# USCCACS/RXMD

Hardware: AMD Instinct MI355X
Metric: MD steps/sec (RDX, 979,776 atoms/GPU; one step advances every GPU's domain: weak scaling, wall-clock steps/s of the whole job) (higher is better)
Workload: dtype f64

## Files before the change

rxmd_amd/csrc/bonded.hip:

```cpp
#include "engine.h"

#include <hipcub/hipcub.hpp>

#include <algorithm>
#include <cstdlib>
#include <type_traits>

namespace rxmd {

static inline int nblk(long long n, int b) { return n > 0 ? static_cast<int>((n + b - 1) / b) : 1; }

static constexpr double MINBO0 = 1e-4, cutof2_esub = 1e-4;
static constexpr double MAXANGLE = 0.999999999999, MINANGLE = -0.999999999999, NSMALL = 1e-10;
static constexpr double PI_ = 3.14159265358979;

__device__ inline double wave_sum_b(double v) { return wave_sum64(v); }
__device__ inline void block_energy_add(double v, double *dst) {
  __shared__ double sm[8];
  v = wave_sum_b(v);
  const int w = threadIdx.x >> 6;
  __syncthreads();
  if ((threadIdx.x & 63) == 0) sm[w] = v;
  __syncthreads();
  if (threadIdx.x == 0) {
// ... 213 lines not shown
        const double BOjk_p4 = pow(BOjk, ap.pval4), exp3jk = exp(-aj.pval3 * BOjk_p4), fn7jk = 1.0 - exp3jk;
        const double exp7 = exp(-ap.pval7 * delta_ang), trm8 = 1.0 + exp6 + exp7;
        const double fn8j = aj.pval5 - (aj.pval5 - 1.0) * (2.0 + exp6) / trm8;
        const double theta0 = PI_ - ap.theta00 * (1.0 - ex10);
        const double theta_diff = theta0 - theta_ijk;
        const double exp2 = exp(-ap.pval2 * theta_diff * theta_diff);
        e5 += fn7ij * fn7jk * fn8j * (ap.pval1 - ap.pval1 * exp2);
        const double Cf7ij = aj.pval3 * ap.pval4 * (BOij_p4 / BOij) * exp3ij;
        const double Cf7jk = aj.pval3 * ap.pval4 * (BOjk_p4 / BOjk) * exp3jk;
        const double Cf8j = (1.0 - aj.pval5) / (trm8 * trm8) * (ff.pval6 * exp6 * trm8 - (2.0 + exp6) * (ff.pval6 * exp6 - ap.pval7 * exp7));
        const double Ctheta0 = ff.pval10 * ap.theta00 * ex10;
        const double CEval1 = Cf7ij * fn7jk * fn8j * ap.pval1 * (1.0 - exp2);
        const double CEval2 = fn7ij * Cf7jk * fn8j * ap.pval1 * (1.0 - exp2);
        const double CEval3 = fn7ij * fn7jk * Cf8j * ap.pval1 * (1.0 - exp2);
        const double CEval4 = 2.0 * ap.pval1 * ap.pval2 * fn7ij * fn7jk * fn8j * exp2 * theta_diff;
        const double CEval5 = CEval4 * Ctheta0 * CSBO2;
        const double CEval6 = CEval5 * dSBO1, CEval7 = CEval5 * dSBO2, CEval8 = CEval4 / sin_ijk;
        const double PEpen = ap.ppen1 * fn9 * epen[oi] * epen[ok];
        e6 += PEpen;
        const double CEpen1 = Cf9j / fn9 * PEpen, CEpen2 = -2.0 * ff.ppen2 * (BOij - 2.0) * PEpen, CEpen3 = -2.0 * ff.ppen2 * (BOjk - 2.0) * PEpen;
        const double sum_BOi = delta[i] + ff.atom[ti].Val, sum_BOk = delta[k] + ff.atom[tk].Val;
        const double ui = -BOij + sum_BOi, uk = -BOjk + sum_BOk;
        const double PEcoa = ap.pcoa1 / (1.0 + exp_coa2) * ecoa[oi] * ecoa[ok];
        e7 += PEcoa;
        const double CEcoa1 = -2.0 * ff.pcoa4 * (BOij - 1.5) * PEcoa, CEcoa2 = -2.0 * ff.pcoa4 * (BOjk - 1.5) * PEcoa;
        const double CEcoa3 = -ff.pcoa2 * exp_coa2 / (1.0 + exp_coa2) * PEcoa;
        const double CEcoa4 = -2.0 * ff.pcoa3 * ui * PEcoa, CEcoa5 = -2.0 * ff.pcoa3 * uk * PEcoa;
        ai_cf += CEpen2 + CEcoa1 - CEcoa4 + CEval1;
        acc1(cf1, l_cf, ok, CEpen3 + CEcoa2 - CEcoa5 + CEval2);
        S_d1 += CEpen1 + CEcoa3 + CEval3 + CEval7; S_v6 += CEval6; S_v5 += CEval5;
        ai_cd += CEcoa4; acc1(cdn, l_cd, ok, CEcoa5);
        V3 fi, fk;
        angle_forces(CEval8, rij, nij, rjk, njk, fi, fk);
        ai_fx += fi.x; ai_fy += fi.y; ai_fz += fi.z;
        acc1(fnx, l_fx, ok, fk.x); acc1(fny, l_fy, ok, fk.y); acc1(fnz, l_fz, ok, fk.z);
        fself.x -= fi.x + fk.x; fself.y -= fi.y + fk.y; fself.z -= fi.z + fk.z;
      }
      if (ai_cf != 0.0) acc1(cf1, l_cf, oi, ai_cf);
      if (ai_cd != 0.0) acc1(cdn, l_cd, oi, ai_cd);
      if (ai_fx != 0.0 || ai_fy != 0.0 || ai_fz != 0.0) { acc1(fnx, l_fx, oi, ai_fx); acc1(fny, l_fy, oi, ai_fy); acc1(fnz, l_fz, oi, ai_fz); }
    }
    if (S_d1 != 0.0 || S_v6 != 0.0 || S_v5 != 0.0)
      for (int n1 = 0; n1 < nj; ++n1) {
        const int o = ob + n1;
        acc1(cf1, l_cf, o, S_d1 + S_v6 * ipow7(bo0[o])); cf2[o] += S_v5; cf3[o] += S_v5;
      }
    fx[j] += fself.x; fy[j] += fself.y; fz[j] += fself.z;
  }
  wave_lds_sync();
  for (int t = lane_; t < nst; t += 64) { cf1[ob_w + t] = l_cf[t]; cdn[ob_w + t] = l_cd[t]; fnx[ob_w + t] = l_fx[t]; fny[ob_w + t] = l_fy[t]; fnz[ob_w + t] = l_fz[t]; }
  block_energy_add(e5, pe + 5); block_energy_add(e6, pe + 6); block_energy_add(e7, pe + 7);
}

constexpr int E3Q_BC = 192;
template <int MINW, int NA>
__global__ void __launch_bounds__(256, MINW) k_e3q(int N, int NG, DevFF ff, const int *__restrict__ boff, const int *__restrict__ nbr, const unsigned char *__restrict__ btype, const int *__restrict__ type,
                                              const double *__restrict__ x, const double *__restrict__ y, const double *__restrict__ z,
                                              const double *__restrict__ bo0, const double *__restrict__ bo2, const double *__restrict__ bo3,
                                              const double *__restrict__ delta, const double *__restrict__ nlp, const double *__restrict__ dDlp,
                                              const double *__restrict__ epen, const double *__restrict__ ecoa,
                                              double *__restrict__ cf1, double *__restrict__ cf2, double *__restrict__ cf3, double *__restrict__ cdn,
                                              double *__restrict__ fnx, double *__restrict__ fny, double *__restrict__ fnz,
                                              double *__restrict__ cds, double *__restrict__ fx, double *__restrict__ fy, double *__restrict__ fz, double *__restrict__ pe, int probe) {
  constexpr int E3Q_NA = NA, E3Q_MAXL = (E3Q_BC / NA < 32) ? E3Q_BC / NA : 32, LPA = 64 / NA;
  __shared__ unsigned char s_ix3[512];
  __shared__ double s_ang[64][7];
  __shared__ double s_c[4][16][12];
  __shared__ int s_ci[4][16][4];
  __shared__ double s_acc[4][5][E3Q_BC];
  __shared__ double s_at[4][16][3];
  __shared__ unsigned char s_cap[4][256], s_own[4][E3Q_BC];
  __shared__ float s_cbo[4][E3Q_BC];
  __shared__ unsigned short s_q[4][128];
  constexpr int CAPW = (256 / NA < 32) ? 256 / NA : 32;
  const int lane = threadIdx.x & 63, w = __builtin_amdgcn_readfirstlane(static_cast<int>(threadIdx.x >> 6));
  for (int t = threadIdx.x; t < ff.n1 * ff.n1 * ff.n1; t += 256) s_ix3[t] = static_cast<unsigned char>(ff.inxn3[t]);
  const bool ang_lds = ff.nvaty <= 63;
  if (ang_lds) for (int t = threadIdx.x; t < 7 * (ff.nvaty + 1); t += 256) s_ang[t / 7][t % 7] = reinterpret_cast<const double *>(ff.angle)[t];
  __syncthreads();
  double e5 = 0.0, e6 = 0.0, e7 = 0.0;
  for (int vb = blockIdx.x; vb < NG; vb += gridDim.x) {
  const int jbase = (xcd_swizzle(vb, NG) * 4 + w) * E3Q_NA;
  if (jbase >= N) continue;
  const int na = min(E3Q_NA, N - jbase);
  const int ob_w = boff[jbase], nb_w = boff[jbase + na] - ob_w;
  for (int r = lane; r < nb_w; r += 64) { s_acc[w][0][r] = bo0[ob_w + r]; s_acc[w][1][r] = bo2[ob_w + r] + bo3[ob_w + r]; }
  for (int t = lane; t < 3 * E3Q_BC; t += 64) (&s_acc[w][2][0])[t] = 0.0;
  if (lane < E3Q_NA) { s_at[w][lane][0] = 0.0; s_at[w][lane][1] = 0.0; s_at[w][lane][2] = 0.0; s_ci[w][lane][2] = 0; s_ci[w][lane][3] = 0; }
  wave_lds_sync();
  if (lane < na) {
    const int j = jbase + lane;
    const int tj = type[j], ob = boff[j], nj = min(boff[j + 1] - ob, E3Q_MAXL);
    const DevAtomP aj = ff.atom[tj];
    double sum_BO8 = 0.0, sum_SBO1 = 0.0;
    int nc = 0;
    for (int n1 = 0; n1 < nj; ++n1) {
      const int r = ob + n1 - ob_w;
      const double b = s_acc[w][0][r], b2 = b * b, b4 = b2 * b2;
      sum_BO8 -= b4 * b4;
      sum_SBO1 += s_acc[w][1][r];
      if (b - cutof2_esub > 0.0) { s_cbo[w][lane * E3Q_MAXL + nc] = static_cast<float>(b); s_cap[w][lane * CAPW + nc++] = static_cast<unsigned char>(n1); }
      s_own[w][r] = static_cast<unsigned char>(lane);
    }
    const double prod_SBO = exp(sum_BO8);
    const double dlj = delta[j];
    const double delta_ang = dlj + aj.Val - aj.Valangle;
    const double nlpj = nlp[j], dDj = dDlp[j];
    const double exp_pen3 = exp(-ff.ppen3 * dlj), exp_pen4 = exp(ff.ppen4 * dlj);
    const double trm34 = 1.0 + exp_pen3 + exp_pen4;
    const double fn9 = (2.0 + exp_pen3) / trm34;
    const double Cf9j = (-ff.ppen3 * exp_pen3 * trm34 - (2.0 + exp_pen3) * (-ff.ppen3 * exp_pen3 + ff.ppen4 * exp_pen4)) / (trm34 * trm34);
    const double delta_val = dlj + aj.Val - aj.Valval;
    const double SBO = sum_SBO1 + (1.0 - prod_SBO) * (-delta_ang - ff.pval8 * nlpj);
    double SBO2 = 0.0, CSBO2 = 0.0;
    if (SBO > 0.0 && SBO <= 1.0) { const double pw = exp(ff.pval9 * log(SBO)); SBO2 = pw; CSBO2 = ff.pval9 * (pw / SBO); }
    else if (SBO > 1.0 && SBO < 2.0) { const double b_ = 2.0 - SBO, pw = exp(ff.pval9 * log(b_)); SBO2 = 2.0 - pw; CSBO2 = ff.pval9 * (pw / b_); }
    else if (SBO >= 2.0) SBO2 = 2.0;
    double *c = s_c[w][lane];
    c[0] = x[j]; c[1] = y[j]; c[2] = z[j]; c[3] = delta_ang; c[4] = exp(ff.pval6 * delta_ang); c[5] = exp(-ff.pval10 * (2.0 - SBO2)); c[6] = CSBO2;
    c[7] = -8.0 * prod_SBO * (delta_ang + ff.pval8 * nlpj); c[8] = (prod_SBO - 1.0) * (1.0 - ff.pval8 * dDj); c[9] = fn9; c[10] = Cf9j / fn9; c[11] = exp(ff.pcoa2 * delta_val);
    s_ci[w][lane][0] = tj; s_ci[w][lane][1] = ob; s_ci[w][lane][2] = nj; s_ci[w][lane][3] = nc;
  }
  wave_lds_sync();
  for (int t = lane; t < 2 * E3Q_BC; t += 64) (&s_acc[w][0][0])[t] = 0.0;
  wave_lds_sync();
  int qn = 0, qh = 0;
  auto evaluate = [&](int cnt) {
#ifdef RXMD_EXPERIMENTS
    if (probe == 2) return;
    if (probe == 5) { if (lane == 0) { atomicAdd(pe + 5, 1.0); atomicAdd(pe + 6, static_cast<double>(cnt)); } return; }
#endif
    if (lane < cnt) {
      const int key = s_q[w][(qh + lane) & 127];
      const int a = key >> 10, i1 = (key >> 5) & 31, k1 = key & 31;
      const double *c = s_c[w][a];
      const int tj = s_ci[w][a][0], ob = s_ci[w][a][1];
      const int oi = ob + i1, ok = ob + k1;
      const double xj = c[0], yj = c[1], zj = c[2], delta_ang = c[3], exp6 = c[4], ex10 = c[5], CSBO2 = c[6], dSBO1 = c[7], dSBO2 = c[8], fn9 = c[9], Cf9j_fn9 = c[10], exp_coa2 = c[11];
      const DevAtomP aj = ff.atom[tj];
      const int i = nbr[oi], ti = btype[oi], k = nbr[ok], tk = btype[ok];
      const double BOij = bo0[oi] - cutof2_esub, BOjk = bo0[ok] - cutof2_esub;
      const V3 rij = {x[i] - xj, y[i] - yj, z[i] - zj};
      const double nij = sqrt(dot(rij, rij));
      const V3 rjk = {xj - x[k], yj - y[k], zj - z[k]};
      const double njk = sqrt(dot(rjk, rjk));
      const int inxn = s_ix3[(ti * ff.n1 + tj) * ff.n1 + tk];
      DevAngleP ap;
      if (ang_lds) { const double *a_ = s_ang[inxn]; ap = DevAngleP{a_[0], a_[1], a_[2], a_[3], a_[4], a_[5], a_[6]}; }
      else ap = ff.angle[inxn];
      double cos_ijk = -dot(rij, rjk) / (nij * njk);
      if (cos_ijk > MAXANGLE) cos_ijk = MAXANGLE;
      if (cos_ijk < MINANGLE) cos_ijk = MINANGLE;
      const double theta_ijk = acos(cos_ijk), sin_ijk = sqrt((1.0 - cos_ijk) * (1.0 + cos_ijk));
      const double BOij_p4 = exp(ap.pval4 * log(BOij)), exp3ij = exp(-aj.pval3 * BOij_p4), fn7ij = 1.0 - exp3ij;
      const double BOjk_p4 = exp(ap.pval4 * log(BOjk)), exp3jk = exp(-aj.pval3 * BOjk_p4), fn7jk = 1.0 - exp3jk;
      const double exp7 = exp(-ap.pval7 * delta_ang), trm8 = 1.0 + exp6 + exp7;
      const double fn8j = aj.pval5 - (aj.pval5 - 1.0) * (2.0 + exp6) / trm8;
      const double theta0 = PI_ - ap.theta00 * (1.0 - ex10);
      const double theta_diff = theta0 - theta_ijk;
      const double exp2 = exp(-ap.pval2 * theta_diff * theta_diff);
      e5 += fn7ij * fn7jk * fn8j * (ap.pval1 - ap.pval1 * exp2);
      const double Cf7ij = aj.pval3 * ap.pval4 * (BOij_p4 / BOij) * exp3ij;
      const double Cf7jk = aj.pval3 * ap.pval4 * (BOjk_p4 / BOjk) * exp3jk;
      const double Cf8j = (1.0 - aj.pval5) / (trm8 * trm8) * (ff.pval6 * exp6 * trm8 - (2.0 + exp6) * (ff.pval6 * exp6 - ap.pval7 * exp7));
      const double Ctheta0 = ff.pval10 * ap.theta00 * ex10;
      const double CEval1 = Cf7ij * fn7jk * fn8j * ap.pval1 * (1.0 - exp2);
      const double CEval2 = fn7ij * Cf7jk * fn8j * ap.pval1 * (1.0 - exp2);
      const double CEval3 = fn7ij * fn7jk * Cf8j * ap.pval1 * (1.0 - exp2);
      const double CEval4 = 2.0 * ap.pval1 * ap.pval2 * fn7ij * fn7jk * fn8j * exp2 * theta_diff;
      const double CEval5 = CEval4 * Ctheta0 * CSBO2;
      const double CEval6 = CEval5 * dSBO1, CEval7 = CEval5 * dSBO2, CEval8 = CEval4 / sin_ijk;
      const double PEpen = ap.ppen1 * fn9 * epen[oi] * epen[ok];
      e6 += PEpen;
      const double CEpen1 = Cf9j_fn9 * PEpen, CEpen2 = -2.0 * ff.ppen2 * (BOij - 2.0) * PEpen, CEpen3 = -2.0 * ff.ppen2 * (BOjk - 2.0) * PEpen;
      const double sum_BOi = delta[i] + ff.atom[ti].Val, sum_BOk = delta[k] + ff.atom[tk].Val;
      const double ui = -BOij + sum_BOi, uk = -BOjk + sum_BOk;
      const double PEcoa = ap.pcoa1 / (1.0 + exp_coa2) * ecoa[oi] * ecoa[ok];
      e7 += PEcoa;
      const double CEcoa1 = -2.0 * ff.pcoa4 * (BOij - 1.5) * PEcoa, CEcoa2 = -2.0 * ff.pcoa4 * (BOjk - 1.5) * PEcoa;
      const double CEcoa3 = -ff.pcoa2 * exp_coa2 / (1.0 + exp_coa2) * PEcoa;
      const double CEcoa4 = -2.0 * ff.pcoa3 * ui * PEcoa, CEcoa5 = -2.0 * ff.pcoa3 * uk * PEcoa;
      V3 fi, fk;
      angle_forces(CEval8, rij, nij, rjk, njk, fi, fk);
      const int ri = oi - ob_w, rk = ok - ob_w;
      atomicAdd(&s_acc[w][0][ri], CEpen2 + CEcoa1 - CEcoa4 + CEval1); atomicAdd(&s_acc[w][1][ri], CEcoa4);
      atomicAdd(&s_acc[w][2][ri], fi.x); atomicAdd(&s_acc[w][3][ri], fi.y); atomicAdd(&s_acc[w][4][ri], fi.z);
      atomicAdd(&s_acc[w][0][rk], CEpen3 + CEcoa2 - CEcoa5 + CEval2); atomicAdd(&s_acc[w][1][rk], CEcoa5);
      atomicAdd(&s_acc[w][2][rk], fk.x); atomicAdd(&s_acc[w][3][rk], fk.y); atomicAdd(&s_acc[w][4][rk], fk.z);
      atomicAdd(&s_at[w][a][0], CEpen1 + CEcoa3 + CEval3 + CEval7); atomicAdd(&s_at[w][a][1], CEval6); atomicAdd(&s_at[w][a][2], CEval5);
    }
    wave_lds_sync();
  };
#ifdef RXMD_EXPERIMENTS
  if (probe == 1) continue;
#endif
  {
    const int a = lane / LPA, sub = lane % LPA;
    const int nc = s_ci[w][a][3], tj = s_ci[w][a][0], ob = s_ci[w][a][1];
    int u = sub, v = sub + 1;
    for (;;) {
      bool live = u < nc - 1;
      const unsigned long long any = __ballot(live);
      if (any == 0ULL) break;
      bool go = false;
      int key = 0;
      if (live) {
        const int i1 = s_cap[w][a * CAPW + u], k1 = s_cap[w][a * CAPW + v];
        const int oi = ob + i1, ok = ob + k1;
        const float pr = s_cbo[w][a * E3Q_MAXL + u] * s_cbo[w][a * E3Q_MAXL + v];
        go = pr > 1.001e-4f;
        if (!go && pr > 0.999e-4f) go = bo0[oi] * bo0[ok] > cutof2_esub;
        if (go) go = s_ix3[(static_cast<int>(btype[oi]) * ff.n1 + tj) * ff.n1 + static_cast<int>(btype[ok])] != 0;
        key = (a << 10) | (i1 << 5) | k1;
        if (++v >= nc) { u += LPA; v = u + 1; }
      }
      const unsigned long long m = __ballot(go);
      if (go) s_q[w][(qh + qn + __popcll(m & ((1ULL << lane) - 1ULL))) & 127] = static_cast<unsigned short>(key);
      qn += __popcll(m);
      wave_lds_sync();
      if (qn >= 64) { evaluate(64); qh = (qh + 64) & 127; qn -= 64; }
    }
    if (qn > 0) evaluate(qn);
  }
  for (int r = lane; r < nb_w; r += 64) {
    const int o = ob_w + r, a = s_own[w][r];
    const double S_d1 = s_at[w][a][0], S_v6 = s_at[w][a][1], S_v5 = s_at[w][a][2];
    const double c1 = s_acc[w][0][r] + (S_d1 + S_v6 * ipow7(bo0[o]));
    if (c1 != 0.0) cf1[o] += c1;
    if (S_v5 != 0.0) { cf2[o] += S_v5; cf3[o] += S_v5; }
    const double cd = s_acc[w][1][r], f0 = s_acc[w][2][r], f1 = s_acc[w][3][r], f2 = s_acc[w][4][r];
    if (cd != 0.0) cdn[o] += cd;
    if (f0 != 0.0 || f1 != 0.0 || f2 != 0.0) { fnx[o] += f0; fny[o] += f1; fnz[o] += f2; }
  }
  if (lane < na) {
    const int j = jbase + lane, r0 = s_ci[w][lane][1] - ob_w, nj = s_ci[w][lane][2];
    double s0 = 0.0, s1 = 0.0, s2 = 0.0;
    for (int t = 0; t < nj; ++t) { s0 += s_acc[w][2][r0 + t]; s1 += s_acc[w][3][r0 + t]; s2 += s_acc[w][4][r0 + t]; }
    if (s0 != 0.0 || s1 != 0.0 || s2 != 0.0) { fx[j] -= s0; fy[j] -= s1; fz[j] -= s2; }
  }
  wave_lds_sync();
  }
  block_energy_add(e5, pe + 5); block_energy_add(e6, pe + 6); block_energy_add(e7, pe + 7);
}

struct BoxImg { double H[9], Hi[9], L[3]; int ortho; int probe; };
template <int LSL, bool ONCE, int WPB>
__global__ void __launch_bounds__(64 * WPB, E4B_MINB) k_e4b(int N, DevFF ff, const int *__restrict__ boff, const int *__restrict__ nbr, const unsigned char *__restrict__ btype, const int *__restrict__ nbrcnt, const int *__restrict__ type,
                                              const long long *__restrict__ gid, const double *__restrict__ x, const double *__restrict__ y, const double *__restrict__ z,
                                              const double *__restrict__ bo0, const double *__restrict__ bo2, const double *__restrict__ delta,
                                              const double *__restrict__ etor, const double *__restrict__ econ,
                                              double *__restrict__ cf1, double *__restrict__ cf2, double *__restrict__ cdn,
                                              double *__restrict__ fnx, double *__restrict__ fny, double *__restrict__ fnz,
                                              double *__restrict__ cds, double *__restrict__ fx, double *__restrict__ fy, double *__restrict__ fz, double *__restrict__ pe, BoxImg bx,
                                              const int *__restrict__ brev, double4 *__restrict__ tkl, unsigned char *__restrict__ tflag, int TW, int VB) {
  __shared__ double s_bo[WPB][64], s_et[WPB][64], s_ec[WPB][64], s_rx[WPB][64], s_ry[WPB][64], s_rz[WPB][64], s_rn[WPB][64];
  __shared__ int s_nb[WPB][64], s_meta[WPB][64];
  __shared__ int s_bofn[WPB][64];
  __shared__ double s_btb2[WPB][64], s_dfn11[WPB][64];
  __shared__ int s_q[WPB][128];
  __shared__ int s_ql[WPB][128]; __shared__ unsigned short s_qx[WPB][128];
  __shared__ int s_cap[WPB][64], s_capl[WPB][64], s_ll[WPB][64], s_tl[WPB][64], s_gj[WPB][8][2];
  __shared__ int s_cb[WPB][64];
  __shared__ int s_cd[WPB][4][9];
  __shared__ int s_base[WPB][9];
  __shared__ double s_bokl[WPB][64];
// ... 619 lines not shown
    for (int c0 = 0; c0 < n; c0 += 256) {
      unsigned ent[4];
#pragma unroll
      for (int u = 0; u < 4; ++u) {
        const int kk = c0 + 64 * u + lane;
        if (SLOTS) {
          ent[u] = 0xffffffffu;
          if (kk < n) {
            const int sl = sl10[row + kk] & 0x7fff;
            const int pos = min(wk[sl / WIN_UNIT] + (sl & (WIN_UNIT - 1)), G - 1);
            ent[u] = static_cast<unsigned>(pos) | (static_cast<unsigned>(stype[pos]) << NB10_IDX_BITS);
          }
        } else ent[u] = kk < n ? static_cast<unsigned>(nb10[row + kk]) : 0xffffffffu;
      }
#pragma unroll
      for (int u = 0; u < 4; ++u) {
        if (c0 + 64 * u >= n) break;
        const int inx = __shfl(inx_l, static_cast<int>((ent[u] >> NB10_IDX_BITS) & 15u), 64);
        const bool keep = ent[u] != 0xffffffffu && inx != 0;
        const unsigned long long m = __ballot(keep);
        if (keep) s_cand[w][qn + __popcll(m & ((1ULL << lane) - 1ULL))] = ent[u];
        qn += __popcll(m);
        if (qn > EHB_CAP - 64) flush();
      }
    }
    if (qn > 0) flush();
    fi_t.x = wave_sum_b(fi_t.x); fi_t.y = wave_sum_b(fi_t.y); fi_t.z = wave_sum_b(fi_t.z);
    if (lane == 0 && (fi_t.x != 0.0 || fi_t.y != 0.0 || fi_t.z != 0.0)) { atomicAdd(fx + i, fi_t.x); atomicAdd(fy + i, fi_t.y); atomicAdd(fz + i, fi_t.z); }
    wave_lds_sync();
  }
  block_energy_add(e10, pe + 10);
}

__global__ void k_zero3(int n, double *__restrict__ a, double *__restrict__ b, double *__restrict__ c) {
  const int k = blockIdx.x * blockDim.x + threadIdx.x;
  if (k < n) { a[k] = 0.0; b[k] = 0.0; c[k] = 0.0; }
}
__global__ void k_add_sorted3(int G, const int *__restrict__ perm, const double *__restrict__ sx, const double *__restrict__ sy, const double *__restrict__ sz,
                              double *__restrict__ fx, double *__restrict__ fy, double *__restrict__ fz) {
  const int k = blockIdx.x * blockDim.x + threadIdx.x;
  if (k >= G) return;
  const double a = sx[k], b = sy[k], c = sz[k];
  if (a != 0.0 || b != 0.0 || c != 0.0) { const int i = perm[k]; fx[i] += a; fy[i] += b; fz[i] += c; }
}

void Engine::bonded_energies() {
  double *pe_d = scal + 32;
  k_ebond_terms<<<nblk(nbonds_res, 256), 256, 0, stream>>>(nbonds_res, dff, bown, nbr, btype, type, gid, bo0, bo1, bo2, bo3, delta, deltalp, cf1, cf2, cf3, ecoa, bt1, bt2, pe_d);
  k_elnpr_atoms<<<nblk(N, 256), 256, 0, stream>>>(N, dff, boff, type, bt1, bt2, delta, deltalp, dDlp, ecoef, pe_d);
  k_elnpr_bonds<<<nblk(nbonds_res, 256), 256, 0, stream>>>(nbonds_res, dff, bown, nbr, btype, type, bo2, bo3, delta, deltalp, dDlp, ecoef, cf1, cf2, cf3, cdn);
  const bool kt3 = kt_begin(&st.ms_k_e3b);
  if (opt.e3b_queue != 0 && dff.n1 <= 8 && dff.nvaty <= 255) {
    const int maxl = h_err[2];
    auto go = [&](auto kern, int na, int minw) {
      const int NG = nblk(N, 4 * na);
      kern<<<std::min(NG, (num_cu * minw + 7) & ~7), 256, 0, stream>>>(N, NG, dff, boff, nbr, btype, type, pos[0], pos[1], pos[2], bo0, bo2, bo3, delta, nlp, dDlp, epen, ecoa, cf1, cf2, cf3, cdn, fnx, fny, fnz,
                                                                     cds, frc[0], frc[1], frc[2], pe_d, static_cast<int>(opt.e4b_probe));
    };
    const bool w3 = opt.e3b_queue == 3;
    if (maxl <= 12) { if (w3) go(k_e3q<3, 16>, 16, 3); else go(k_e3q<2, 16>, 16, 2); }
    else if (maxl <= 24) { if (w3) go(k_e3q<3, 8>, 8, 3); else go(k_e3q<2, 8>, 8, 2); }
    else { if (w3) go(k_e3q<3, 4>, 4, 3); else go(k_e3q<2, 4>, 4, 2); }
  } else
    k_e3b<<<nblk(N, 256), 256, 4 * 5 * E3B_CAP * sizeof(double), stream>>>(N, dff, boff, nbr, btype, type, pos[0], pos[1], pos[2], bo0, bo2, bo3, delta, nlp, dDlp, epen, ecoa, cf1, cf2, cf3, cdn, fnx, fny, fnz,
                                          cds, frc[0], frc[1], frc[2], pe_d);
  RX_HIP(hipGetLastError());
  kt_end(kt3);
  BoxImg bx;
  for (int a = 0; a < 3; ++a) { for (int c = 0; c < 3; ++c) { bx.H[3 * a + c] = box.H[a][c]; bx.Hi[3 * a + c] = box.Hi[a][c]; } bx.L[a] = box.lat[a]; }
  bx.ortho = grid.ortho; bx.probe = 0;
  bx.probe = static_cast<int>(opt.e4b_probe);
  const int want = static_cast<int>(opt.e4b_slots);
  const bool narrow = h_err[2] <= 15 && want != 32 && want != 4;
  const bool kt4 = kt_begin(&st.ms_k_e4b);
  bool once = opt.e4b_once != 0;
  const int TW = (std::max(h_err[2], 8) + 3) & ~3;
  if (once) {
    const size_t need = static_cast<size_t>(std::max(nbonds, 1)) * TW;
    if (need > e4b_cap) {
      size_t fre = 0, tot = 0;
      RX_HIP(hipMemGetInfo(&fre, &tot));
      const size_t want_entries = need + need / 4;
      if (want_entries * 33 > (fre + e4b_cap * 33) / 2) once = false; else alloc_e4b_delivery(want_entries);
    }
  }
  if (once) {
    if (e4b_dirty) RX_HIP(hipMemsetAsync(e4b_flag, 0, e4b_cap, stream));
    e4b_dirty = true;
  }
  const int n4 = dff.n1 * dff.n1 * dff.n1 * dff.n1;
  const size_t tor_bytes = (dff.n1 <= 8 && dff.ntoty <= 255) ? static_cast<size_t>((n4 + 15) & ~15) : 0;
  const bool wpb1 = opt.e4b_wpb == 1;
  auto launch = [&](auto inst, int per_wave) {
    constexpr int L = decltype(inst)::value;
    auto go = [&](auto kern, int wpb) {
      const int VB = nblk(N, per_wave * wpb);
      const int grid = opt.e4b_persist != 0 ? std::min(VB, (num_cu * (12 / wpb) + 7) & ~7) : VB;
      kern<<<grid, 64 * wpb, tor_bytes, stream>>>(N, dff, boff, nbr, btype, nbrcnt, type, gid, pos[0], pos[1], pos[2], bo0, bo2, delta, etor, econ, cf1, cf2, cdn, fnx, fny, fnz,
                                                  cds, frc[0], frc[1], frc[2], pe_d, bx, brev, e4b_t, e4b_flag, TW, VB);
    };
    if (once) { if (wpb1) go(k_e4b<L, true, 1>, 1); else go(k_e4b<L, true, 4>, 4); }
    else      { if (wpb1) go(k_e4b<L, false, 1>, 1); else go(k_e4b<L, false, 4>, 4); }
    RX_HIP(hipGetLastError());
  };
  if (want == 4) launch(std::integral_constant<int, 1>{}, 4);
  else if (narrow && want != 16) launch(std::integral_constant<int, 0>{}, 8);
  else if (narrow) launch(std::integral_constant<int, 4>{}, 4);
  else launch(std::integral_constant<int, 5>{}, 2);
  if (once) {
    k_e4b_deliver<<<nblk(nbonds, 256), 256, 0, stream>>>(nbonds, TW, e4b_t, reinterpret_cast<unsigned *>(e4b_flag), cf1, fnx, fny, fnz);
    e4b_dirty = false;
  }
  kt_end(kt4);
  const bool kth = kt_begin(&st.ms_k_ehb);
  if (ehb_donor_types != 0u) {
// ... 35 lines not shown
```

rxmd_amd/csrc/buffers.hip:

```cpp
#include "engine.h"

#include <algorithm>
#include <cstring>
#include <utility>

namespace rxmd {

static const Options g_opt = Options::from_env();
static const bool g_poison = g_opt.poison_alloc;
#ifdef RXMD_EXPERIMENTS
static const long long g_contig = g_opt.contig_alloc;
#endif

bool poison_enabled() { return g_poison; }

void *dev_alloc(size_t bytes, Fill fill) {
  void *p = nullptr;
#ifdef RXMD_EXPERIMENTS
  if (fill == Fill::Pattern && (g_contig == 0 || (g_contig > 0 && bytes <= static_cast<size_t>(g_contig)))) RX_HIP(hipExtMallocWithFlags(&p, bytes, hipDeviceMallocContiguous));
  else
#endif
  RX_HIP(hipMalloc(&p, bytes));
  if (fill != Fill::None && hipMemset(p, fill == Fill::Pattern && g_poison ? 0xFF : 0, bytes) != hipSuccess) {
    (void)hipFree(p);
// ... 41 lines not shown
  b.add(hst, G_SETUP, Dim::NB, 1, 0, P, ghosts, res);
  b.add(gst, G_SETUP, Dim::NB, 1, 0, P, ghosts, res);
  b.add(hst2, G_SETUP, Dim::NB, 1, 0, P, ghosts);
  b.add(tickets, G_SETUP, Dim::Fixed, 0, 16, Z, never);
  b.add(sall, G_SETUP, Dim::Rows10, 1, 0, P, whole);
  b.add(sgh, G_SETUP, Dim::Rows10, 1, 0, P, whole);
  b.add(wall, G_SETUP, Dim::Rows10, 1, 0, P, whole);
  b.add(wgh, G_SETUP, Dim::Rows10, 1, 0, P, whole);
  b.add(gsrc, G_SETUP, Dim::NB, 1, 0, P, whole);
  b.add(groot, G_SETUP, Dim::NB, 1, 0, P, whole);
  b.add(gowner, G_SETUP, Dim::NB, 1, 0, P, never);
  b.add(dh_ghost, G_SETUP, Dim::NB, 1, 0, P, never);
  b.add(dh_keys, G_SETUP, Dim::NB, 1, 0, P, never);
  b.add(dh_keys2, G_SETUP, Dim::NB, 1, 0, P, never);
  b.add(dh_vals, G_SETUP, Dim::NB, 1, 0, P, never);
  b.add(dh_off, G_SETUP, Dim::Fixed, 0, 1100, P, never);
  b.add(sendidx, G_SETUP, Dim::NB, 1, 0, P, never);
  b.add(rootperm, G_SETUP, Dim::NB, 1, 0, P, whole);
  b.add(invpos, G_SETUP, Dim::NB, 1, 0, P, whole);
  b.add(xs, G_SETUP, Dim::NB, 1, 0, P, whole);
  for (int a = 0; a < 3; ++a) {
    b.add(fnb[a], G_SETUP, Dim::NB, 1, 0, P, never);
    b.add(fsort[a], G_SETUP, Dim::NB, 1, 0, P, never);
  }
  b.add(cellid, G_SETUP, Dim::NB, 1, 0, P, whole);
  b.add(cellid_sorted, G_SETUP, Dim::NB, 1, 0, P, whole);
  b.add(perm, G_SETUP, Dim::NB, 1, 0, P, whole);
  b.add(perm_in, G_SETUP, Dim::NB, 1, 0, P, whole);
  b.add(cellstart, G_CELLSTART, Dim::Cap, 1, 0, P, whole);
  b.add(sorted_xyzi, G_SETUP, Dim::NB, 1, 0, P, whole);
  b.add(sorted_type, G_SETUP, Dim::NB, 1, 0, P, whole);
  b.add(flags, G_SETUP, Dim::NB, 1, 1, P, whole);
  b.add(scanout, G_SETUP, Dim::NB, 1, 1, P, whole);
  b.add(flags2, G_SETUP, Dim::NB, 1, 1, P, whole);
  b.add(scanout2, G_SETUP, Dim::NB, 1, 1, P, whole);
  b.add(nbr_sm, G_SETUP, Dim::NB, 32, 0, P, whole);
  b.add(nbrcnt, G_SETUP, Dim::NB, 1, 1, P, whole);
  b.add(boff, G_SETUP, Dim::NB, 1, 2, P, whole);
  b.add(nbr, G_BOND, Dim::Cap, 1, 0, P, whole);
  b.add(brev, G_BOND, Dim::Cap, 1, 0, P, whole);
  b.add(bown, G_BOND, Dim::Cap, 1, 0, P, whole);
  b.add(btype, G_BOND, Dim::Cap, 1, 0, P, whole);
  for (double **t : {&bo0, &bo1, &bo2, &bo3, &dln2, &dln3, &dBOp, &A0, &A1, &A2, &A3, &cf1, &cf2, &cf3, &cdn, &fnx, &fny, &fnz, &etor, &econ, &epen, &ecoa, &bt1, &bt2, &bt3})
    b.add(*t, G_BOND, Dim::Cap, 1, 0, P, whole);
  b.add(ehb_don, G_SETUP, Dim::Rows10, 1, EHB_DON_EXTRA, P, whole);
  b.add(ehb_cnt, G_SETUP, Dim::Fixed, 0, 72, Z, never);
  b.add(ecoef, G_SETUP, Dim::NB, 6, 0, P, whole);
  b.add(deltap, G_SETUP, Dim::NB, 1, 0, P, whole);
  b.add(delta, G_SETUP, Dim::NB, 1, 0, P, whole);
  b.add(nlp, G_SETUP, Dim::NB, 1, 0, P, whole);
  b.add(dDlp, G_SETUP, Dim::NB, 1, 0, P, whole);
  b.add(deltalp, G_SETUP, Dim::NB, 1, 0, P, whole);
  b.add(cds, G_SETUP, Dim::NB, 1, 0, P, whole);
  b.add(cd, G_SETUP, Dim::NB, 1, 0, P, whole);
  b.add(cc_, G_SETUP, Dim::NB, 1, 0, P, whole);
  b.add(nb10, G_LIST10, Dim::List10, 1, 0, P, whole);
  b.add(rows_int, G_SETUP, Dim::Rows10, 1, 0, P, whole);
  b.add(rows_bnd, G_SETUP, Dim::Rows10, 1, 0, P, whole);
  b.add(hess, G_LIST10, Dim::List10, 1, 0, P, whole);
  b.add(n10, G_SETUP, Dim::Rows10, 1, 0, P, whole);
  for (double2 **t : {&r_qst, &r_hst, &r_hst2, &r_gst, &r_sall, &r_sgh, &r_wall, &r_wgh}) b.add(*t, G_WIN, Dim::Cap, WIN_ROWS, 0, P, never);
  b.add(r_type, G_WIN, Dim::Cap, WIN_ROWS, 0, P, never);
  b.add(r_n10, G_WIN, Dim::Cap, WIN_ROWS, 0, P, never);
  b.add(r_xpos, G_WIN, Dim::Cap, WIN_ROWS, 0, P, never);
  b.add(rpos, G_WIN, Dim::NB, 1, 0, P, never);
  b.add(g_rrow, G_WIN, Dim::NB, 1, 0, P, never);
  b.add(rows_sorted, G_WIN, Dim::Cap, WIN_ROWS, 0, P, whole);
  b.add(rowcols, G_WIN, Dim::Cap, WIN_ROWS * 64, 0, P, whole);
  b.add(grp_base, G_WIN, Dim::Cap, 32, 0, P, whole);
  b.add(win_flag, G_WIN, Dim::Cap, 1, 1, P, whole);
  b.add(win_k, G_WIN, Dim::Cap, WIN_MAXUNITS, 0, P, whole);
  b.add(win_cnt, G_WIN, Dim::Cap, 1, 0, P, whole);
  b.add(win_gint, G_WIN, Dim::Cap, 1, 0, P, whole);
  b.add(win_gbnd, G_WIN, Dim::Cap, 1, 0, P, whole);
  b.add(sl10, G_LIST10, Dim::List10, 1, 0, P, whole);
  b.add(partials, G_PARTIALS, Dim::Cap, 1, 1024, P, whole);
  b.add(scal, G_SETUP, Dim::Fixed, 0, SCAL_N, Z, never, res);
  b.add_pinned(h_scal, G_SETUP, H_SCAL_DOUBLES, true);
  b.add(tsum, G_SETUP, Dim::Fixed, 0, 128, Z, never);
  b.add_raw(reinterpret_cast<void **>(&sargs), sizeof(double), G_SETUP, Dim::Fixed, 0, 32, Z, never);
  b.add(d_err, G_SETUP, Dim::Fixed, 0, 16, Z, never);
  b.add_pinned(h_err, G_SETUP, H_ERR_INTS, false);
  b.add(cubtmp, G_CUBTMP, Dim::Cap, 1, 0, Fill::None, never);
  b.add(ffblob, G_FFBLOB, Dim::Cap, 1, 0, Fill::None, never);
  b.add(pqblob, G_PQBLOB, Dim::Cap, 1, 0, Fill::None, never);
  b.add(e4b_t, G_E4B, Dim::Cap, 1, 0, P, never);
  b.add(e4b_flag, G_E4B, Dim::Cap, 1, 0, Z, never);
  b.add(seg_cnt, G_SEG, Dim::Cap, 27, 0, P, never);
  b.add(seg_tot, G_SEG, Dim::Fixed, 0, 32, Z, never);
  b.add(seg_code_, G_SEG, Dim::Cap, 256, 0, P, never);
  b.add_pinned(h_seg, G_SEG_PINNED, H_SEG_INTS, false);
  b.add_pinned(h_pub, G_SEG_PINNED, H_PUB_WORDS, true);
  b.add(xbuf_send, G_XBUF, Dim::Cap, 1, 0, P, whole);
  b.add(xbuf_recv, G_XBUF, Dim::Cap, 1, 0, P, whole);
  b.add(dh_serve, G_DH_SERVE, Dim::Cap, 1, 0, P, never);
}

size_t Buffers::count(const Buf &b, const Engine &e) const {
  size_t d = 0;
  switch (b.dim) {
    case Dim::Fixed: break;
    case Dim::NB: d = static_cast<size_t>(e.NB); break;
    case Dim::Rows10: d = static_cast<size_t>(e.rows10); break;
    case Dim::List10: d = static_cast<size_t>(e.rows10) * e.S10; break;
    case Dim::Cap: d = cap[b.group]; break;
  }
// ... 61 lines not shown
```

rxmd_amd/csrc/engine.h:

```cpp
#pragma once
#include <hip/hip_runtime.h>

#include <string>
#include <type_traits>
#include <vector>

#include "../../include/rxmd_hip.h"
#include "ffparams.h"
#include "options.h"

namespace rxmd {

#define RX_HIP(call)                                                                              \
  do {                                                                                            \
    hipError_t e_ = (call);                                                                       \
    if (e_ != hipSuccess) throw EngineError(RXMD_E_HIP, std::string(#call) + ": " + hipGetErrorString(e_)); \
  } while (0)

struct EngineError {
  int code;
  std::string msg;
  EngineError(int c, std::string m) : code(c), msg(std::move(m)) {}
};

// ... 146 lines not shown
  int max_row10 = 0, min_row10 = 0;
  int num_cu = 256;
  int N = 0, G = 0, copyptr[7] = {0};
  int cc[3] = {1, 1, 1};
  double shell[3] = {0, 0, 0};
  Grid grid{};
  RefMesh rmesh{};

  Buffers bufs;
  void declare_buffers();
  DevFF dff{};
  void *ffblob = nullptr, *pqblob = nullptr;
  double *pos[3] = {}, *vel[3] = {}, *frc[3] = {}, *spos[3] = {};
  double *q = nullptr, *qsfp = nullptr, *qsfv = nullptr;
  double *shl[3] = {}; double4 *sorted_shl = nullptr; double *hsc = nullptr; double4 *pqrow = nullptr;
  int *type = nullptr; long long *gid = nullptr;
  double2 *qst = nullptr, *hst = nullptr, *gst = nullptr;
  double2 *hst2 = nullptr;
  unsigned *tickets = nullptr;
  double2 *sall = nullptr, *sgh = nullptr, *wall = nullptr, *wgh = nullptr;
  int *gsrc = nullptr, *groot = nullptr;
  int *rootperm = nullptr;
  int *invpos = nullptr;
  double2 *xs = nullptr;
  int *sendidx = nullptr; int sendoff[8] = {0};
  int *cellid = nullptr, *cellid_sorted = nullptr, *perm = nullptr, *perm_in = nullptr, *cellstart = nullptr;
  double4 *sorted_xyzi = nullptr;
  unsigned char *sorted_type = nullptr;
  bool nb10_valid = false, nb10_sticky = false;
  bool needs_nb10(bool selfcheck) const;
  bool sorted_w_charge = false;
  void sorted_positions();
  void sorted_charge_only();
  void require_nb10();
  bool list_selfcheck = false;
  void *cubtmp = nullptr; size_t cubtmp_bytes = 0;
  int *flags = nullptr, *scanout = nullptr;
  int *nbr = nullptr, *nbrcnt = nullptr, *boff = nullptr, *brev = nullptr, *bown = nullptr;
  unsigned char *btype = nullptr;
  int *nbr_sm = nullptr;
  size_t bcap = 0; int nbonds = 0;
  void alloc_bond_tables(size_t cap); void free_bond_tables();
  double *bo0 = nullptr, *bo1 = nullptr, *bo2 = nullptr, *bo3 = nullptr, *dln2 = nullptr, *dln3 = nullptr, *dBOp = nullptr;
  double *A0 = nullptr, *A1 = nullptr, *A2 = nullptr, *A3 = nullptr;
  double *cf1 = nullptr, *cf2 = nullptr, *cf3 = nullptr, *cdn = nullptr, *fnx = nullptr, *fny = nullptr, *fnz = nullptr;
  double *etor = nullptr, *econ = nullptr, *epen = nullptr, *ecoa = nullptr;
  double *bt1 = nullptr, *bt2 = nullptr, *bt3 = nullptr;
  double *ecoef = nullptr;
  double4 *e4b_t = nullptr; unsigned char *e4b_flag = nullptr; size_t e4b_cap = 0; bool e4b_dirty = false;
  void alloc_e4b_delivery(size_t entries);
  int nbonds_res = 0;
  int2 *ehb_don = nullptr; size_t ehb_don_cap = 0; int *ehb_cnt = nullptr; unsigned ehb_donor_types = 0u; int ehb_blocks_per_cu = 0, ehb_blocks_per_cu_sl = 0;
  double *deltap = nullptr, *delta = nullptr, *nlp = nullptr, *dDlp = nullptr, *deltalp = nullptr;
  double *cds = nullptr, *cd = nullptr, *cc_ = nullptr;
  int *nb10 = nullptr, *n10 = nullptr; double *hess = nullptr;
  size_t partials_cap = 0;
  double *partials = nullptr;
  double *scal = nullptr;
  double *h_scal = nullptr;
  int *d_err = nullptr, *h_err = nullptr, *h_cnt = nullptr;
  double *xbuf_send = nullptr, *xbuf_recv = nullptr; size_t xbuf_doubles = 0; bool xbuf_owned = false;
  double pe[14] = {0}, astr[6] = {0};

  hipStream_t stream = nullptr;
  hipStream_t comm_stream = nullptr; hipEvent_t ev_main = nullptr, ev_comm = nullptr, ev_est = nullptr, ev_pass[2][2] = {{nullptr, nullptr}, {nullptr, nullptr}};
  template <class F> void on_comm_stream(F &&body) {
    RX_HIP(hipEventRecord(ev_main, stream));
    RX_HIP(hipStreamWaitEvent(comm_stream, ev_main, 0));
    std::swap(stream, comm_stream);
    in_comm_region = true;
    try { body(); } catch (...) { in_comm_region = false; std::swap(stream, comm_stream); throw; }
    in_comm_region = false;
    std::swap(stream, comm_stream);
    RX_HIP(hipEventRecord(ev_comm, comm_stream));
  }
  bool in_comm_region = false;
  hipStream_t bond_stream = nullptr; hipEvent_t ev_fork = nullptr, ev_bond = nullptr;
  double *fsort[3] = {nullptr, nullptr, nullptr};
  double *fnb[3] = {nullptr, nullptr, nullptr};
  bool bond_overlap() const { return bond_stream != nullptr && !ff.pqeq; }
  void bonded_chain_begin();
  void join_comm_stream() { const bool kt = kt_begin(&st.ms_halo_exposed, nullptr, nullptr, 2); RX_HIP(hipStreamWaitEvent(stream, ev_comm, 0)); kt_end(kt); }
  hipEvent_t ev[8] = {};
  std::vector<double> last_atype, last_pos[3];
  std::vector<double> lex_p, lex_v; bool lex_pending = false;
  rxmd_stats st{};
  int nstep_qeq = 0; double last_est = 0;
  std::vector<double> est_trace;
  double atype_resid = 0.0;
  long long step_count = 0;
  unsigned long long velocity_draws = 0;

  explicit Engine(const rxmd_config &c);
  ~Engine();
  void kinetic_and_charge(double &ke, double &qsum);
  void set_atoms_rxff(int natoms, const double *rec10);
  void set_atoms_arrays(int natoms, const double *atype, const double *x, const double *y, const double *z, const double *q, const double *lexp, const double *lexv);
  int get_atoms_rxff(double *rec10, int capacity);
  void build_ghosts_and_lists(bool qeq_prepass = false);
  void qeq_start_vectors();
  int *rows_int = nullptr, *rows_bnd = nullptr; int n_bnd = 0; bool rows_split_pending = false;
  bool rows_split_pending_invalid() const { return n_bnd < 0 || n_bnd > N; }
  bool sums_from_list = false;
  void qeq();
  void force(bool defer_host_read = false, bool observe_energy = true);
  void finish_force();
// ... 166 lines not shown
```

Measured before the change: 23.82.

## Precompute e3 centre records in a prepass and cache per-bond geometry in LDS

Moves the per-centre atom terms (SBO, penalty and coalition factors, coordinates) of the three-body queue kernel into a separate one-thread-per-atom kernel that writes a 12-double record plus a bond cutoff bitmask per atom. The queue kernel loads these records and caches per-bond vectors, lengths, log(BO) and bond types in LDS, so each angle evaluation no longer recomputes sqrt/log or gathers positions and btype from global memory. The e3b_queue==3 occupancy variant is dropped and min waves fixed at 2. It adds an extra kernel launch, a global buffer round trip and a larger LDS footprint per block, which can lower occupancy.

```diff
diff --git a/rxmd_amd/csrc/bonded.hip b/rxmd_amd/csrc/bonded.hip
--- a/rxmd_amd/csrc/bonded.hip
+++ b/rxmd_amd/csrc/bonded.hip
@@ -289,12 +289,50 @@
   block_energy_add(e5, pe + 5); block_energy_add(e6, pe + 6); block_energy_add(e7, pe + 7);
 }
 
+__global__ void __launch_bounds__(256) k_e3_centres(int N, DevFF ff, const int *__restrict__ boff, const int *__restrict__ type,
+                                                    const double *__restrict__ x, const double *__restrict__ y, const double *__restrict__ z,
+                                                    const double *__restrict__ bo0, const double *__restrict__ bo2, const double *__restrict__ bo3,
+                                                    const double *__restrict__ delta, const double *__restrict__ nlp, const double *__restrict__ dDlp,
+                                                    double *__restrict__ rec, unsigned *__restrict__ qmask) {
+  const int j = blockIdx.x * blockDim.x + threadIdx.x;
+  if (j >= N) return;
+  const int tj = type[j], ob = boff[j], nj = min(boff[j + 1] - ob, 32);
+  const DevAtomP aj = ff.atom[tj];
+  double sum_BO8 = 0.0, sum_SBO1 = 0.0;
+  unsigned m = 0u;
+  for (int n1 = 0; n1 < nj; ++n1) {
+    const double b = bo0[ob + n1], b2 = b * b, b4 = b2 * b2;
+    sum_BO8 -= b4 * b4;
+    sum_SBO1 += bo2[ob + n1] + bo3[ob + n1];
+    if (b - cutof2_esub > 0.0) m |= 1u << n1;
+  }
+  const double prod_SBO = exp(sum_BO8);
+  const double dlj = delta[j];
+  const double delta_ang = dlj + aj.Val - aj.Valangle;
+  const double nlpj = nlp[j], dDj = dDlp[j];
+  const double exp_pen3 = exp(-ff.ppen3 * dlj), exp_pen4 = exp(ff.ppen4 * dlj);
+  const double trm34 = 1.0 + exp_pen3 + exp_pen4;
+  const double fn9 = (2.0 + exp_pen3) / trm34;
+  const double Cf9j = (-ff.ppen3 * exp_pen3 * trm34 - (2.0 + exp_pen3) * (-ff.ppen3 * exp_pen3 + ff.ppen4 * exp_pen4)) / (trm34 * trm34);
+  const double delta_val = dlj + aj.Val - aj.Valval;
+  const double SBO = sum_SBO1 + (1.0 - prod_SBO) * (-delta_ang - ff.pval8 * nlpj);
+  double SBO2 = 0.0, CSBO2 = 0.0;
+  if (SBO > 0.0 && SBO <= 1.0) { const double pw = exp(ff.pval9 * log(SBO)); SBO2 = pw; CSBO2 = ff.pval9 * (pw / SBO); }
+  else if (SBO > 1.0 && SBO < 2.0) { const double b_ = 2.0 - SBO, pw = exp(ff.pval9 * log(b_)); SBO2 = 2.0 - pw; CSBO2 = ff.pval9 * (pw / b_); }
+  else if (SBO >= 2.0) SBO2 = 2.0;
+  double2 *c = reinterpret_cast<double2 *>(rec + 12 * static_cast<size_t>(j));
+  c[0] = make_double2(x[j], y[j]); c[1] = make_double2(z[j], delta_ang); c[2] = make_double2(exp(ff.pval6 * delta_ang), exp(-ff.pval10 * (2.0 - SBO2)));
+  c[3] = make_double2(CSBO2, -8.0 * prod_SBO * (delta_ang + ff.pval8 * nlpj)); c[4] = make_double2((prod_SBO - 1.0) * (1.0 - ff.pval8 * dDj), fn9);
+  c[5] = make_double2(Cf9j / fn9, exp(ff.pcoa2 * delta_val));
+  qmask[j] = m;
+}
+
 constexpr int E3Q_BC = 192;
-template <int MINW, int NA>
-__global__ void __launch_bounds__(256, MINW) k_e3q(int N, int NG, DevFF ff, const int *__restrict__ boff, const int *__restrict__ nbr, const unsigned char *__restrict__ btype, const int *__restrict__ type,
+template <int NA>
+__global__ void __launch_bounds__(256, 2) k_e3q(int N, int NG, DevFF ff, const int *__restrict__ boff, const int *__restrict__ nbr, const unsigned char *__restrict__ btype, const int *__restrict__ type,
                                               const double *__restrict__ x, const double *__restrict__ y, const double *__restrict__ z,
-                                              const double *__restrict__ bo0, const double *__restrict__ bo2, const double *__restrict__ bo3,
-                                              const double *__restrict__ delta, const double *__restrict__ nlp, const double *__restrict__ dDlp,
+                                              const double *__restrict__ bo0, const double *__restrict__ rec, const unsigned *__restrict__ qmask,
+                                              const double *__restrict__ delta,
                                               const double *__restrict__ epen, const double *__restrict__ ecoa,
                                               double *__restrict__ cf1, double *__restrict__ cf2, double *__restrict__ cf3, double *__restrict__ cdn,
                                               double *__restrict__ fnx, double *__restrict__ fny, double *__restrict__ fnz,
@@ -309,6 +347,8 @@
   __shared__ unsigned char s_cap[4][256], s_own[4][E3Q_BC];
   __shared__ float s_cbo[4][E3Q_BC];
   __shared__ unsigned short s_q[4][128];
+  __shared__ double s_geo[4][5][E3Q_BC];
+  __shared__ unsigned char s_bt[4][E3Q_BC];
   constexpr int CAPW = (256 / NA < 32) ? 256 / NA : 32;
   const int lane = threadIdx.x & 63, w = __builtin_amdgcn_readfirstlane(static_cast<int>(threadIdx.x >> 6));
   for (int t = threadIdx.x; t < ff.n1 * ff.n1 * ff.n1; t += 256) s_ix3[t] = static_cast<unsigned char>(ff.inxn3[t]);
@@ -321,45 +361,36 @@
   if (jbase >= N) continue;
   const int na = min(E3Q_NA, N - jbase);
   const int ob_w = boff[jbase], nb_w = boff[jbase + na] - ob_w;
-  for (int r = lane; r < nb_w; r += 64) { s_acc[w][0][r] = bo0[ob_w + r]; s_acc[w][1][r] = bo2[ob_w + r] + bo3[ob_w + r]; }
-  for (int t = lane; t < 3 * E3Q_BC; t += 64) (&s_acc[w][2][0])[t] = 0.0;
+  for (int r = lane; r < nb_w; r += 64) s_acc[w][0][r] = bo0[ob_w + r];
+  for (int t = lane; t < 12 * na; t += 64) (&s_c[w][0][0])[t] = rec[12 * static_cast<size_t>(jbase) + t];
+  for (int t = lane; t < 4 * E3Q_BC; t += 64) (&s_acc[w][1][0])[t] = 0.0;
   if (lane < E3Q_NA) { s_at[w][lane][0] = 0.0; s_at[w][lane][1] = 0.0; s_at[w][lane][2] = 0.0; s_ci[w][lane][2] = 0; s_ci[w][lane][3] = 0; }
   wave_lds_sync();
   if (lane < na) {
     const int j = jbase + lane;
     const int tj = type[j], ob = boff[j], nj = min(boff[j + 1] - ob, E3Q_MAXL);
-    const DevAtomP aj = ff.atom[tj];
-    double sum_BO8 = 0.0, sum_SBO1 = 0.0;
+    unsigned m = qmask[j];
+    if (nj < 32) m &= (1u << nj) - 1u;
     int nc = 0;
-    for (int n1 = 0; n1 < nj; ++n1) {
-      const int r = ob + n1 - ob_w;
-      const double b = s_acc[w][0][r], b2 = b * b, b4 = b2 * b2;
-      sum_BO8 -= b4 * b4;
-      sum_SBO1 += s_acc[w][1][r];
-      if (b - cutof2_esub > 0.0) { s_cbo[w][lane * E3Q_MAXL + nc] = static_cast<float>(b); s_cap[w][lane * CAPW + nc++] = static_cast<unsigned char>(n1); }
-      s_own[w][r] = static_cast<unsigned char>(lane);
-    }
-    const double prod_SBO = exp(sum_BO8);
-    const double dlj = delta[j];
-    const double delta_ang = dlj + aj.Val - aj.Valangle;
-    const double nlpj = nlp[j], dDj = dDlp[j];
-    const double exp_pen3 = exp(-ff.ppen3 * dlj), exp_pen4 = exp(ff.ppen4 * dlj);
-    const double trm34 = 1.0 + exp_pen3 + exp_pen4;
-    const double fn9 = (2.0 + exp_pen3) / trm34;
-    const double Cf9j = (-ff.ppen3 * exp_pen3 * trm34 - (2.0 + exp_pen3) * (-ff.ppen3 * exp_pen3 + ff.ppen4 * exp_pen4)) / (trm34 * trm34);
-    const double delta_val = dlj + aj.Val - aj.Valval;
-    const double SBO = sum_SBO1 + (1.0 - prod_SBO) * (-delta_ang - ff.pval8 * nlpj);
-    double SBO2 = 0.0, CSBO2 = 0.0;
-    if (SBO > 0.0 && SBO <= 1.0) { const double pw = exp(ff.pval9 * log(SBO)); SBO2 = pw; CSBO2 = ff.pval9 * (pw / SBO); }
-    else if (SBO > 1.0 && SBO < 2.0) { const double b_ = 2.0 - SBO, pw = exp(ff.pval9 * log(b_)); SBO2 = 2.0 - pw; CSBO2 = ff.pval9 * (pw / b_); }
-    else if (SBO >= 2.0) SBO2 = 2.0;
-    double *c = s_c[w][lane];
-    c[0] = x[j]; c[1] = y[j]; c[2] = z[j]; c[3] = delta_ang; c[4] = exp(ff.pval6 * delta_ang); c[5] = exp(-ff.pval10 * (2.0 - SBO2)); c[6] = CSBO2;
-    c[7] = -8.0 * prod_SBO * (delta_ang + ff.pval8 * nlpj); c[8] = (prod_SBO - 1.0) * (1.0 - ff.pval8 * dDj); c[9] = fn9; c[10] = Cf9j / fn9; c[11] = exp(ff.pcoa2 * delta_val);
+    for (int n1 = 0; n1 < nj; ++n1) s_own[w][ob + n1 - ob_w] = static_cast<unsigned char>(lane);
+    while (m) {
+      const int n1 = __ffs(m) - 1;
+      m &= m - 1u;
+      s_cbo[w][lane * E3Q_MAXL + nc] = static_cast<float>(s_acc[w][0][ob + n1 - ob_w]); s_cap[w][lane * CAPW + nc++] = static_cast<unsigned char>(n1);
+    }
     s_ci[w][lane][0] = tj; s_ci[w][lane][1] = ob; s_ci[w][lane][2] = nj; s_ci[w][lane][3] = nc;
   }
   wave_lds_sync();
-  for (int t = lane; t < 2 * E3Q_BC; t += 64) (&s_acc[w][0][0])[t] = 0.0;
+  for (int r = lane; r < nb_w; r += 64) {
+    const int o = ob_w + r, i = nbr[o];
+    const double *c = s_c[w][s_own[w][r]];
+    const double b = s_acc[w][0][r];
+    const V3 rij = {x[i] - c[0], y[i] - c[1], z[i] - c[2]};
+    s_geo[w][0][r] = rij.x; s_geo[w][1][r] = rij.y; s_geo[w][2][r] = rij.z; s_geo[w][3][r] = sqrt(dot(rij, rij));
+    if (b - cutof2_esub > 0.0) s_geo[w][4][r] = log(b - cutof2_esub);
+    s_bt[w][r] = btype[o];
+    s_acc[w][0][r] = 0.0;
+  }
   wave_lds_sync();
   int qn = 0, qh = 0;
   auto evaluate = [&](int cnt) {
@@ -373,14 +404,16 @@
       const double *c = s_c[w][a];
       const int tj = s_ci[w][a][0], ob = s_ci[w][a][1];
       const int oi = ob + i1, ok = ob + k1;
-      const double xj = c[0], yj = c[1], zj = c[2], delta_ang = c[3], exp6 = c[4], ex10 = c[5], CSBO2 = c[6], dSBO1 = c[7], dSBO2 = c[8], fn9 = c[9], Cf9j_fn9 = c[10], exp_coa2 = c[11];
+      const double delta_ang = c[3], exp6 = c[4], ex10 = c[5], CSBO2 = c[6], dSBO1 = c[7], dSBO2 = c[8], fn9 = c[9], Cf9j_fn9 = c[10], exp_coa2 = c[11];
       const DevAtomP aj = ff.atom[tj];
-      const int i = nbr[oi], ti = btype[oi], k = nbr[ok], tk = btype[ok];
+      const int ri = oi - ob_w, rk = ok - ob_w;
       const double BOij = bo0[oi] - cutof2_esub, BOjk = bo0[ok] - cutof2_esub;
-      const V3 rij = {x[i] - xj, y[i] - yj, z[i] - zj};
-      const double nij = sqrt(dot(rij, rij));
-      const V3 rjk = {xj - x[k], yj - y[k], zj - z[k]};
-      const double njk = sqrt(dot(rjk, rjk));
+      const int i = nbr[oi], ti = s_bt[w][ri], k = nbr[ok], tk = s_bt[w][rk];
+      const V3 rij = {s_geo[w][0][ri], s_geo[w][1][ri], s_geo[w][2][ri]};
+      const double nij = s_geo[w][3][ri];
+      const V3 rjk = {-s_geo[w][0][rk], -s_geo[w][1][rk], -s_geo[w][2][rk]};
+      const double njk = s_geo[w][3][rk];
+      const double ln_ij = s_geo[w][4][ri], ln_jk = s_geo[w][4][rk];
       const int inxn = s_ix3[(ti * ff.n1 + tj) * ff.n1 + tk];
       DevAngleP ap;
       if (ang_lds) { const double *a_ = s_ang[inxn]; ap = DevAngleP{a_[0], a_[1], a_[2], a_[3], a_[4], a_[5], a_[6]}; }
@@ -389,8 +422,8 @@
       if (cos_ijk > MAXANGLE) cos_ijk = MAXANGLE;
       if (cos_ijk < MINANGLE) cos_ijk = MINANGLE;
       const double theta_ijk = acos(cos_ijk), sin_ijk = sqrt((1.0 - cos_ijk) * (1.0 + cos_ijk));
-      const double BOij_p4 = exp(ap.pval4 * log(BOij)), exp3ij = exp(-aj.pval3 * BOij_p4), fn7ij = 1.0 - exp3ij;
-      const double BOjk_p4 = exp(ap.pval4 * log(BOjk)), exp3jk = exp(-aj.pval3 * BOjk_p4), fn7jk = 1.0 - exp3jk;
+      const double BOij_p4 = exp(ap.pval4 * ln_ij), exp3ij = exp(-aj.pval3 * BOij_p4), fn7ij = 1.0 - exp3ij;
+      const double BOjk_p4 = exp(ap.pval4 * ln_jk), exp3jk = exp(-aj.pval3 * BOjk_p4), fn7jk = 1.0 - exp3jk;
       const double exp7 = exp(-ap.pval7 * delta_ang), trm8 = 1.0 + exp6 + exp7;
       const double fn8j = aj.pval5 - (aj.pval5 - 1.0) * (2.0 + exp6) / trm8;
       const double theta0 = PI_ - ap.theta00 * (1.0 - ex10);
@@ -419,7 +452,6 @@
       const double CEcoa4 = -2.0 * ff.pcoa3 * ui * PEcoa, CEcoa5 = -2.0 * ff.pcoa3 * uk * PEcoa;
       V3 fi, fk;
       angle_forces(CEval8, rij, nij, rjk, njk, fi, fk);
-      const int ri = oi - ob_w, rk = ok - ob_w;
       atomicAdd(&s_acc[w][0][ri], CEpen2 + CEcoa1 - CEcoa4 + CEval1); atomicAdd(&s_acc[w][1][ri], CEcoa4);
       atomicAdd(&s_acc[w][2][ri], fi.x); atomicAdd(&s_acc[w][3][ri], fi.y); atomicAdd(&s_acc[w][4][ri], fi.z);
       atomicAdd(&s_acc[w][0][rk], CEpen3 + CEcoa2 - CEcoa5 + CEval2); atomicAdd(&s_acc[w][1][rk], CEcoa5);
@@ -447,7 +479,7 @@
         const float pr = s_cbo[w][a * E3Q_MAXL + u] * s_cbo[w][a * E3Q_MAXL + v];
         go = pr > 1.001e-4f;
         if (!go && pr > 0.999e-4f) go = bo0[oi] * bo0[ok] > cutof2_esub;
-        if (go) go = s_ix3[(static_cast<int>(btype[oi]) * ff.n1 + tj) * ff.n1 + static_cast<int>(btype[ok])] != 0;
+        if (go) go = s_ix3[(static_cast<int>(s_bt[w][oi - ob_w]) * ff.n1 + tj) * ff.n1 + static_cast<int>(s_bt[w][ok - ob_w])] != 0;
         key = (a << 10) | (i1 << 5) | k1;
         if (++v >= nc) { u += LPA; v = u + 1; }
       }
@@ -1173,15 +1205,15 @@
   const bool kt3 = kt_begin(&st.ms_k_e3b);
   if (opt.e3b_queue != 0 && dff.n1 <= 8 && dff.nvaty <= 255) {
     const int maxl = h_err[2];
-    auto go = [&](auto kern, int na, int minw) {
+    k_e3_centres<<<nblk(N, 256), 256, 0, stream>>>(N, dff, boff, type, pos[0], pos[1], pos[2], bo0, bo2, bo3, delta, nlp, dDlp, e3c, e3m);
+    auto go = [&](auto kern, int na) {
       const int NG = nblk(N, 4 * na);
-      kern<<<std::min(NG, (num_cu * minw + 7) & ~7), 256, 0, stream>>>(N, NG, dff, boff, nbr, btype, type, pos[0], pos[1], pos[2], bo0, bo2, bo3, delta, nlp, dDlp, epen, ecoa, cf1, cf2, cf3, cdn, fnx, fny, fnz,
+      kern<<<std::min(NG, (num_cu * 2 + 7) & ~7), 256, 0, stream>>>(N, NG, dff, boff, nbr, btype, type, pos[0], pos[1], pos[2], bo0, e3c, e3m, delta, epen, ecoa, cf1, cf2, cf3, cdn, fnx, fny, fnz,
                                                                      cds, frc[0], frc[1], frc[2], pe_d, static_cast<int>(opt.e4b_probe));
     };
-    const bool w3 = opt.e3b_queue == 3;
-    if (maxl <= 12) { if (w3) go(k_e3q<3, 16>, 16, 3); else go(k_e3q<2, 16>, 16, 2); }
-    else if (maxl <= 24) { if (w3) go(k_e3q<3, 8>, 8, 3); else go(k_e3q<2, 8>, 8, 2); }
-    else { if (w3) go(k_e3q<3, 4>, 4, 3); else go(k_e3q<2, 4>, 4, 2); }
+    if (maxl <= 12) go(k_e3q<16>, 16);
+    else if (maxl <= 24) go(k_e3q<8>, 8);
+    else go(k_e3q<4>, 4);
   } else
     k_e3b<<<nblk(N, 256), 256, 4 * 5 * E3B_CAP * sizeof(double), stream>>>(N, dff, boff, nbr, btype, type, pos[0], pos[1], pos[2], bo0, bo2, bo3, delta, nlp, dDlp, epen, ecoa, cf1, cf2, cf3, cdn, fnx, fny, fnz,
                                           cds, frc[0], frc[1], frc[2], pe_d);
diff --git a/rxmd_amd/csrc/buffers.hip b/rxmd_amd/csrc/buffers.hip
--- a/rxmd_amd/csrc/buffers.hip
+++ b/rxmd_amd/csrc/buffers.hip
@@ -117,6 +117,8 @@
   b.add(dDlp, G_SETUP, Dim::NB, 1, 0, P, whole);
   b.add(deltalp, G_SETUP, Dim::NB, 1, 0, P, whole);
   b.add(cds, G_SETUP, Dim::NB, 1, 0, P, whole);
+  b.add(e3c, G_SETUP, Dim::NB, 12, 0, P, whole);
+  b.add(e3m, G_SETUP, Dim::NB, 1, 0, P, whole);
   b.add(cd, G_SETUP, Dim::NB, 1, 0, P, whole);
   b.add(cc_, G_SETUP, Dim::NB, 1, 0, P, whole);
   b.add(nb10, G_LIST10, Dim::List10, 1, 0, P, whole);
diff --git a/rxmd_amd/csrc/engine.h b/rxmd_amd/csrc/engine.h
--- a/rxmd_amd/csrc/engine.h
+++ b/rxmd_amd/csrc/engine.h
@@ -222,6 +222,7 @@
   int nbonds_res = 0;
   int2 *ehb_don = nullptr; size_t ehb_don_cap = 0; int *ehb_cnt = nullptr; unsigned ehb_donor_types = 0u; int ehb_blocks_per_cu = 0, ehb_blocks_per_cu_sl = 0;
   double *deltap = nullptr, *delta = nullptr, *nlp = nullptr, *dDlp = nullptr, *deltalp = nullptr;
+  double *e3c = nullptr; unsigned *e3m = nullptr;
   double *cds = nullptr, *cd = nullptr, *cc_ = nullptr;
   int *nb10 = nullptr, *n10 = nullptr; double *hess = nullptr;
   size_t partials_cap = 0;
```

Result: no change. 23.84 (median of 4 runs) (+0.1%).
